# philres/ngmlr

Measured on AMD Instinct MI355X. Metric: aligned Gbp/hour (PacBio 10kb synthetic, convex-gap SW hot path, host buffers in -> results out, CIGAR bit-exact), higher is better.
Workload: dtype f32

## Files before the change

### include/cvx_align.h

```cpp
#ifndef CVX_ALIGN_H
#define CVX_ALIGN_H

#include <stdint.h>
#include <stddef.h>

#ifdef __cplusplus
extern "C" {
#endif

#define CVX_ABI_VERSION 9

enum {
	CVX_OK = 0,
	CVX_ERR_NO_DEVICE = -1,
	CVX_ERR_PARAMS = -2,
	CVX_ERR_ARG = -3,
	CVX_ERR_OOM = -4,
	CVX_ERR_HIP = -5,
	CVX_ERR_CAPACITY = -6
};

enum {
	CVX_TILE_OK = 0,
	CVX_TILE_INVALID_ROW0 = 1,
// ... 109 lines not shown

int cvx_batch_upload(cvx_handle h, int32_t n_tiles, const cvx_tile *tiles, cvx_batch *out);
int cvx_batch_run(cvx_handle h, cvx_batch b);
int cvx_batch_timing(cvx_batch b, cvx_timing *t);
int cvx_batch_ops_total(cvx_batch b, uint64_t *n_ops);
int cvx_batch_launch_info(cvx_batch b, int32_t i, cvx_launch_info *info);
int cvx_batch_download(cvx_handle h, cvx_batch b, cvx_result *results,
		uint32_t *ops_arena, uint64_t ops_capacity, uint64_t *ops_used);
void cvx_batch_free(cvx_handle h, cvx_batch b);

int cvx_submit(cvx_handle h, int32_t n_tiles, const cvx_tile *tiles, cvx_job *out);
int cvx_wait(cvx_handle h, cvx_job job, const cvx_result **results, const uint32_t **ops, uint64_t *n_ops);
int cvx_job_poll(cvx_handle h, cvx_job job, int32_t *done);
int cvx_job_timing(cvx_job job, cvx_timing *t);
int cvx_job_launch_info(cvx_job job, int32_t i, cvx_launch_info *info);
void cvx_job_release(cvx_handle h, cvx_job job);

int cvx_host_alloc(uint64_t bytes, void **out);
void cvx_host_free(void *p);

int cvx_corridor_rows(cvx_handle h, const cvx_tile *tile, int32_t *offset, int32_t *length);

int cvx_pack_probe(int32_t n_tiles, const cvx_tile *tiles, int32_t iters, int32_t assume_page_locked, double *ms_per_iter, uint64_t *bytes_touched);

typedef struct cvx_genome_s *cvx_genome;
uint64_t cvx_genome_encoded_bytes(int32_t n, const uint64_t *lengths);
int cvx_genome_encode(int32_t n, const char *const *seqs, const uint64_t *lengths, uint8_t *bin_ref,
		uint64_t *n_nibbles, uint64_t *start_table, int32_t *n_starts);
int cvx_genome_upload(cvx_handle h, const uint8_t *bin_ref, uint64_t n_nibbles, const uint64_t *start_table,
		int32_t n_starts, cvx_genome *out);
// ... 173 lines not shown
```

### ngmlr_amd/capi.py

```python
from __future__ import annotations

import ctypes as C
import os

HERE = os.path.dirname(os.path.abspath(__file__))
LIB_PATH = os.environ.get("CVX_LIB") or os.path.join(HERE, "libcvxalign.so")

CVX_OK = 0
STAGE_SCORE, STAGE_DECODE, STAGE_SEARCH = 0, 1, 2
ERR_NAMES = {0: "CVX_OK", -1: "CVX_ERR_NO_DEVICE", -2: "CVX_ERR_PARAMS", -3: "CVX_ERR_ARG",
             -4: "CVX_ERR_OOM", -5: "CVX_ERR_HIP", -6: "CVX_ERR_CAPACITY"}
TILE_STATUS = {0: "ok", 1: "invalid-row0", 2: "invalid-edge", 3: "invalid-length", 4: "too-large",
               5: "empty", -1: "unsupported"}

EXPORTS = ("cvx_last_error", "cvx_abi_version", "cvx_source_id", "cvx_device_count", "cvx_device_synchronize", "cvx_create", "cvx_destroy",
           "cvx_align_batch", "cvx_batch_upload", "cvx_batch_run", "cvx_batch_timing",
           "cvx_batch_ops_total", "cvx_batch_launch_info", "cvx_batch_download", "cvx_batch_free",
           "cvx_submit", "cvx_wait", "cvx_job_timing", "cvx_job_launch_info", "cvx_job_release",
           "cvx_format_alignment", "cvx_format_batch", "cvx_score_batch",
           "cvx_genome_encoded_bytes", "cvx_genome_encode", "cvx_genome_upload", "cvx_genome_free",
           "cvx_genome_decode", "cvx_submit_windows", "cvx_job_text",
           "cvx_host_alloc", "cvx_host_free", "cvx_corridor_rows", "cvx_pack_probe", "cvx_build_id", "cvx_job_poll", "cvx_score_kernel_ms",
           "cvx_index_upload", "cvx_index_free", "cvx_search_batch", "cvx_search_batch_ex", "cvx_job_nm_profile", "cvx_job_nm_profile_resident", "cvx_job_text_all", "cvx_job_window_refs", "cvx_job_nm_sizes", "cvx_nm_profile_ops",
           "cvx_job_nm_regions", "cvx_nm_regions_ops", "cvx_nm_regions_host",
           "cvx_sam_record_text", "cvx_sam_unmapped_text", "cvx_sam_batch", "cvx_stage_kernel_ms", "cvx_search_last_attempts", "cvx_index_build", "cvx_index_build_device",
           "cvx_corridor_fit", "cvx_corridor_fit_batch", "cvx_create_ex", "cvx_runtime_regime", "cvx_search_batch_arena",
           "cvx_score_submit", "cvx_score_poll", "cvx_score_wait")


class CvxParams(C.Structure):
    _fields_ = [("match", C.c_float), ("mismatch", C.c_float), ("gap_open", C.c_float),
                ("gap_extend", C.c_float), ("gap_extend_min", C.c_float), ("gap_decay", C.c_float)]

# ... 114 lines not shown
    lib.cvx_batch_upload.argtypes = [C.c_void_p, C.c_int32, C.POINTER(CvxTile), C.POINTER(C.c_void_p)]
    lib.cvx_batch_run.argtypes = [C.c_void_p, C.c_void_p]
    lib.cvx_batch_timing.argtypes = [C.c_void_p, C.POINTER(CvxTiming)]
    lib.cvx_batch_launch_info.argtypes = [C.c_void_p, C.c_int32, C.POINTER(CvxLaunchInfo)]
    lib.cvx_batch_ops_total.argtypes = [C.c_void_p, C.POINTER(C.c_uint64)]
    lib.cvx_batch_download.argtypes = [C.c_void_p, C.c_void_p, C.POINTER(CvxResult), C.c_void_p,
                                       C.c_uint64, C.POINTER(C.c_uint64)]
    lib.cvx_batch_free.argtypes = [C.c_void_p, C.c_void_p]
    lib.cvx_batch_free.restype = None
    lib.cvx_submit.argtypes = [C.c_void_p, C.c_int32, C.POINTER(CvxTile), C.POINTER(C.c_void_p)]
    lib.cvx_wait.argtypes = [C.c_void_p, C.c_void_p, C.POINTER(C.POINTER(CvxResult)), C.POINTER(C.POINTER(C.c_uint32)),
                             C.POINTER(C.c_uint64)]
    lib.cvx_job_poll.argtypes = [C.c_void_p, C.c_void_p, C.POINTER(C.c_int32)]
    lib.cvx_job_timing.argtypes = [C.c_void_p, C.POINTER(CvxTiming)]
    lib.cvx_job_launch_info.argtypes = [C.c_void_p, C.c_int32, C.POINTER(CvxLaunchInfo)]
    lib.cvx_job_release.argtypes = [C.c_void_p, C.c_void_p]
    lib.cvx_job_release.restype = None
    lib.cvx_format_batch.argtypes = [C.c_int32, C.POINTER(CvxResult), C.c_void_p, C.POINTER(CvxTile),
                                     C.POINTER(CvxTextBuffers), C.POINTER(CvxAlignmentText), C.c_int32]
    lib.cvx_genome_encoded_bytes.restype = C.c_uint64
    lib.cvx_genome_encoded_bytes.argtypes = [C.c_int32, C.c_void_p]
    lib.cvx_genome_encode.argtypes = [C.c_int32, C.POINTER(C.c_char_p), C.c_void_p, C.c_void_p, C.POINTER(C.c_uint64),
                                      C.c_void_p, C.POINTER(C.c_int32)]
    lib.cvx_genome_upload.argtypes = [C.c_void_p, C.c_void_p, C.c_uint64, C.c_void_p, C.c_int32, C.POINTER(C.c_void_p)]
    lib.cvx_genome_free.argtypes = [C.c_void_p, C.c_void_p]
    lib.cvx_genome_free.restype = None
    lib.cvx_genome_decode.argtypes = [C.c_void_p, C.c_void_p, C.c_int32, C.c_void_p, C.c_void_p, C.c_void_p, C.c_void_p]
    lib.cvx_submit_windows.argtypes = [C.c_void_p, C.c_void_p, C.c_int32, C.POINTER(CvxTile), C.c_void_p, C.POINTER(C.c_void_p)]
    lib.cvx_job_text.argtypes = [C.c_void_p, C.c_void_p, C.c_void_p, C.c_void_p, C.POINTER(CvxAlignmentText), C.c_void_p,
                                 C.POINTER(C.c_char_p), C.POINTER(C.c_uint64)]
# ... 67 lines not shown
```

### ngmlr_amd/csrc/cvx_host_logic.h

```cpp
#ifndef CVX_HOST_LOGIC_H
#define CVX_HOST_LOGIC_H

#include <algorithm>
#include <cmath>
#include <condition_variable>
#include <cstdlib>
#include <cstring>
#include <deque>
#include <functional>
#include <mutex>
#include <system_error>
#include <thread>
#include <vector>

#include <pthread.h>

#include "cvx_align.h"
#include "cvx_types.h"

namespace cvx {


struct KernelClass {
	int m;
// ... 523 lines not shown
		hp.n_fast++;
		hp.cls[(size_t) k * 2 + (wrap ? 1 : 0)].push_back(i);
	}
	for (size_t slot = 0; slot < per_tile.size(); ++slot) {
		size_t deepest = 0;
		for (auto &v : per_tile[slot]) deepest = std::max(deepest, v.size());
		for (size_t g = 0; g < deepest; ++g)
			for (auto &v : per_tile[slot])
				if (g < v.size()) hp.chain_tasks[slot].push_back(v[g]);
	}
	for (auto &v : hp.cls) lpt_sort(v, plan);
}



struct ScheduleTuning {
	int exact_steps = kExactDirectSteps;
	int bt_group = 0;
	bool bt_per_class = true;
	bool overlap_post = false;
	int wide_prio = 1, gang_prio = 0, chain_prio = -1, chain_lds_kb = 48;
};

enum { kModeTwoPhase = 0, kModeExact = 1, kModeChain = 2 };

enum StreamSlot { kOnSide0 = 0, kOnPost = 1, kOnMain = 2, kOnSide1 = 3, kStreamSlots = 4 };

struct WalkPlan { int n_long = 0, long_lanes = 32, bulk_lanes = 64; };

inline WalkPlan walk_plan(int count, int n_walk, int bt_group, uint64_t mean_h, const int32_t *list, const TileIn *tin) {
	const int auto_group = count <= 6144 ? 64 : count <= 12288 ? 32 : count <= 49152 ? 16 : 8;
	WalkPlan w;
	w.bulk_lanes = bt_group > 0 ? bt_group : bt_group < 0 ? (n_walk < 4096 ? 64 : 8) : auto_group;
	if (bt_group <= 0 && w.bulk_lanes <= 16)
		while (w.n_long < count && (uint64_t) tin[(size_t) list[w.n_long]].H > 3 * mean_h) w.n_long++;
	return w;
}

inline size_t chain_pad_lds(uint64_t live, int num_cus, int chain_lds_kb, bool rings_beside) {
	const uint64_t resident = std::min<uint64_t>(8192, std::max<uint64_t>(768, live + live / 2 + 256));
	const size_t per_cu = (size_t) ((resident + (uint64_t) num_cus - 1) / (uint64_t) num_cus);
	size_t pad_lds = per_cu >= 32 ? 0 : (size_t) (160 * 1024) / per_cu - 4096;
	pad_lds = std::min<size_t>(pad_lds, 60 * 1024) / 256 * 256;
	if (rings_beside && chain_lds_kb > 0 && per_cu > 0 && per_cu < 32) {
		const size_t budget = (size_t) chain_lds_kb * 1024 / per_cu;
		const size_t capped = budget > 4096 ? (budget - 4096) / 256 * 256 : 0;
		pad_lds = std::min(pad_lds, capped);
	}
	return pad_lds;
}

// ... 7 lines not shown
	size_t pad_lds = 0;
	int prio = 0;
	int stream = kOnMain;
	size_t bt_off = 0;
	int bt_count = 0;
	WalkPlan walk;
	cvx_launch_info info;
};

struct ComputeSchedule {
	std::vector<FillLaunch> launches;
	size_t n_listed = 0;
	size_t bt_begin = 0;
	int n_walk = 0;
	bool per_class = false;
	WalkPlan walk;
	size_t chain_task_off[kNumChainClasses * 2] = {0}, chain_tile_off[kNumChainClasses * 2] = {0};
	size_t chain_blk_off = 0, chain_bytes = 0;
};

inline void build_schedule(HostPlan &hp, const TilePlan *plan, const TileIn *tin, int n, uint64_t n_rows, int num_cus,
		const ScheduleTuning &t, int32_t *lists, ComputeSchedule &s) {
	size_t n_listed = 0;
	size_t cls_off[kNumClasses * 2];
	int n_direct[kNumClasses * 2];
	int ring_classes = 0;
	for (size_t c = 0; c < hp.cls.size(); ++c) {
		std::vector<int32_t> &v = hp.cls[c];
		cls_off[c] = n_listed;
		n_direct[c] = 0;
// ... 69 lines not shown
			const TileIn &in = tin[(size_t) ti];
			L.info.cells += p.cells; L.info.active_cells += p.active;
			L.info.alg_bytes += p.cells + 6ull * (uint64_t) in.H + 2ull * (uint64_t) in.W;
			L.info.read_bases += (uint64_t) in.H;
			if (!hp.trun[(size_t) ti].skip) count[(size_t) bucket(ti) + 1]++;
		}
		for (int k = 0; k < kBuckets; ++k) count[(size_t) k + 1] += count[(size_t) k];
		L.bt_off = n_listed;
		L.bt_count = count[(size_t) kBuckets];
		for (int32_t ti : *L.tiles) if (!hp.trun[(size_t) ti].skip) lists[n_listed + (size_t) count[(size_t) bucket(ti)]++] = ti;
		n_listed += (size_t) L.bt_count;
	}
	s.n_listed = n_listed;
	s.n_walk = (int) (n_listed - s.bt_begin);

	s.per_class = t.bt_per_class && s.launches.size() > 1 && !t.overlap_post && s.n_walk >= 4096;
	const uint64_t mean_h = n_rows / (uint64_t) std::max(n, 1);
	if (s.per_class) for (FillLaunch &L : s.launches) L.walk = walk_plan(L.bt_count, s.n_walk, t.bt_group, mean_h, lists + L.bt_off, tin);
	else s.walk = walk_plan(s.n_walk, s.n_walk, t.bt_group, mean_h, lists + s.bt_begin, tin);

	s.chain_blk_off = s.chain_bytes = 0;
	if (hp.n_chained) {
		for (size_t c = 0; c < hp.chain_tasks.size(); ++c) { s.chain_task_off[c] = s.chain_bytes; s.chain_bytes += hp.chain_tasks[c].size() * sizeof(ChainTask); }
		s.chain_blk_off = s.chain_bytes; s.chain_bytes += hp.chain_blk.size() * sizeof(ChainBlk);
		for (size_t c = 0; c < hp.chain_tiles.size(); ++c) { s.chain_tile_off[c] = s.chain_bytes; s.chain_bytes += (hp.chain_tiles[c].size() * sizeof(int32_t) + 7) / 8 * 8; }
	}
}

}

#endif
```

### ngmlr_amd/csrc/cvx_rt.h

```cpp
#ifndef CVX_RT_H
#define CVX_RT_H

#include <hip/hip_runtime_api.h>

#include <atomic>
#include <cstdint>
#include <mutex>
#include <string>
#include <vector>

#include "cvx_align.h"
#include "cvx_host_logic.h"
#include "cvx_launch.h"
#include "cvx_nm_regions.h"
#include "cvx_rt_err.h"
#include "cvx_types.h"

using namespace cvx;

#define HIP_TRY(expr)                                                              \
	do {                                                                           \
		hipError_t e_ = (expr);                                                    \
		if (e_ != hipSuccess) {                                                    \
			set_err("%s failed: %s (%s:%d)", #expr, hipGetErrorString(e_), __FILE__, __LINE__); \
			return (e_ == hipErrorOutOfMemory) ? CVX_ERR_OOM : CVX_ERR_HIP;        \
		}                                                                          \
	} while (0)

// ... 178 lines not shown
	bool have_refs = false;
	DevBuf<WindowDesc> d_win;
	PinBuf h_chain;
	DevBuf<uint8_t> d_chain;
	DevBuf<BoundaryRec> d_bnd;
	uint32_t bnd_epoch = 0;
	DevBuf<ChainOut> d_chain_out;

	hipEvent_t ev_bt0 = nullptr, ev_bt1 = nullptr;
	hipEvent_t ev_in = nullptr;
	hipEvent_t ev_res = nullptr;
	hipEvent_t ev[5] = {nullptr, nullptr, nullptr, nullptr, nullptr};
	std::vector<hipEvent_t> lev;
	std::vector<cvx_launch_info> launches;
	cvx_timing timing;

	const TileIn *tin() const { return h_tin.as<TileIn>(); }
	const TilePlan *plan() const { return h_plan.as<TilePlan>(); }
	const ResultRec *res() const { return h_res.as<ResultRec>(); }
	const BatchSummary *summary() const { return reinterpret_cast<const BatchSummary *>(h_res.as<uint8_t>() + (size_t) n * sizeof(ResultRec)); }

	static const int kSharedMarks = 32;
	void bind(size_t *marks) {
		int k = 0;
		PinBuf *pins[] = { &h_seq, &h_delta, &h_rsrc, &h_tin, &h_plan, &h_trun, &h_tout, &h_lists, &h_res, &h_ops, &h_chain };
		for (PinBuf *b_ : pins) b_->hwm = &marks[k++];
		d_seq.hwm = &marks[k++]; d_rows.hwm = &marks[k++]; d_delta.hwm = &marks[k++]; d_rsrc.hwm = &marks[k++]; d_tin.hwm = &marks[k++];
		d_plan.hwm = &marks[k++]; d_trun.hwm = &marks[k++]; d_tout.hwm = &marks[k++]; d_dirs.hwm = &marks[k++]; d_regions.hwm = &marks[k++];
		d_lists.hwm = &marks[k++]; d_dstoff.hwm = &marks[k++]; d_dense.hwm = &marks[k++]; d_res.hwm = &marks[k++];
		d_chain.hwm = &marks[k++]; d_bnd.hwm = &marks[k++]; d_chain_out.hwm = &marks[k++];
// ... 29 lines not shown
		if (ev_res) { (void) hipEventDestroy(ev_res); ev_res = nullptr; }
		if (ev_bt0) { (void) hipEventDestroy(ev_bt0); ev_bt0 = nullptr; }
		if (ev_bt1) { (void) hipEventDestroy(ev_bt1); ev_bt1 = nullptr; }
		for (auto &e : ev) if (e) { (void) hipEventDestroy(e); e = nullptr; }
		for (auto &e : lev) if (e) (void) hipEventDestroy(e);
		lev.clear();
	}
};

struct cvx_context {
	int device = 0;
	hipStream_t s_io = nullptr;
	hipStream_t s_main = nullptr;
	hipStream_t s_text = nullptr;
	hipStream_t s_post = nullptr;
	hipStream_t aux[kAuxStreams] = {nullptr};
	bool service = false;
	bool owns_main = true;
	std::mutex streams_mtx;
	std::atomic<bool> streams_ready{false};
	hipStream_t s_main2 = nullptr, s_post2 = nullptr, aux2[kAuxStreams] = {nullptr};
	unsigned small_jobs = 0;
	ScoreParams sp;
	uint64_t max_matrix_mb = 10000;
	int num_cus = 256;
	int pack_threads = 16;
	int tune_min_slots = 0;
	int tune_late_min = kLateMinGroups;
	int tune_late_shift = kLateShift;
	int tune_max_slots = 0;
// ... 1 lines not shown
	int tune_gang_prio = 0;
	int tune_gangs = 0;
	int tune_long_steps = 0, tune_small_batch = 0;
	bool single_lane = true;
	int tune_exact_steps = kExactDirectSteps;
	int tune_wide_prio = 1;
	int tune_chain_prio = -1;
	int tune_chain_lds_kb = 48;
	int tune_chain_m = 0;
	int tune_force_wrap = 0;
	int tune_pen_table = 1;
	int test_fail_compute = 0;
	int bt_group = 0;
	bool bt_per_class = true;
	bool overlap_post = false;
	bool sse_variant = false;
	size_t marks[cvx_batch_s::kSharedMarks] = {0};
	std::vector<cvx_batch_s *> pool;
	std::vector<cvx_batch_s *> pending;
	std::vector<cvx_batch_s *> live;
	float decode_kernel_ms = 0.0f;
	bool score_no_diag = false;
	struct cvx_score_state *score = nullptr;
	struct cvx_search_state *search = nullptr;
};

struct cvx_genome_s {
	int device = 0;
	uint64_t n_nibbles = 0;
	int32_t n_starts = 0;
// ... 6 lines not shown
```

### ngmlr_amd/csrc/cvx_rt_align.cpp

```cpp
#include <algorithm>
#include <atomic>
#include <chrono>
#include <cstdio>
#include <cstdlib>
#include <cstring>
#include <new>
#include <string>
#include <vector>

#include "cvx_rt.h"

namespace {

static const size_t kPoolBatches = 8;

cvx_batch_s *acquire_batch(cvx_context *h) {
	if (!h->pool.empty()) {
		cvx_batch_s *b = h->pool.back();
		h->pool.pop_back();
		return b;
	}
	return new (std::nothrow) cvx_batch_s();
}

// ... 244 lines not shown
	a.sp = h->sp;
	ba.chain_blk = chain_blk;
	ba.n_tiles = b->n;
}

int issue_walk(cvx_batch_s *b, const BacktrackArgs &ba, const WalkPlan &w, size_t at, int count, hipStream_t ws, hipStream_t side) {
	if (count <= 0) return CVX_OK;
	const int32_t *list = b->d_lists.p + at;
	const bool fork = w.n_long > 0 && side != nullptr;
	if (fork) {
		HIP_TRY(hipEventRecord(b->ev_bt0, ws));
		HIP_TRY(hipStreamWaitEvent(side, b->ev_bt0, 0));
	}
	if (w.n_long > 0) HIP_TRY(launch_backtrack(ba, list, w.n_long, w.long_lanes, fork ? side : ws));
	if (fork) HIP_TRY(hipEventRecord(b->ev_bt1, side));
	HIP_TRY(launch_backtrack(ba, list + w.n_long, count - w.n_long, w.bulk_lanes, ws));
	if (fork) HIP_TRY(hipStreamWaitEvent(ws, b->ev_bt1, 0));
	return CVX_OK;
}

int upload_chain(cvx_batch_s *b, const HostPlan &hp, const ComputeSchedule &sch, hipStream_t st) {
	RC_TRY(b->h_chain.ensure(sch.chain_bytes));
	uint8_t *hc = b->h_chain.as<uint8_t>();
	for (size_t c = 0; c < hp.chain_tasks.size(); ++c)
		if (!hp.chain_tasks[c].empty()) memcpy(hc + sch.chain_task_off[c], hp.chain_tasks[c].data(), hp.chain_tasks[c].size() * sizeof(ChainTask));
	memcpy(hc + sch.chain_blk_off, hp.chain_blk.data(), hp.chain_blk.size() * sizeof(ChainBlk));
	for (size_t c = 0; c < hp.chain_tiles.size(); ++c)
		if (!hp.chain_tiles[c].empty()) memcpy(hc + sch.chain_tile_off[c], hp.chain_tiles[c].data(), hp.chain_tiles[c].size() * sizeof(int32_t));
	RC_TRY(b->d_chain.ensure(sch.chain_bytes));
	RC_TRY(b->d_chain_out.ensure(hp.chain_blk.size()));
	{
		const size_t had = b->d_bnd.cap;
		RC_TRY(b->d_bnd.ensure((size_t) hp.bnd_recs + 64));
		if (b->d_bnd.cap != had || b->bnd_epoch >= kBndEpochMax) {
			HIP_TRY(hipMemsetAsync(b->d_bnd.p, 0, b->d_bnd.cap * sizeof(BoundaryRec), st));
			b->bnd_epoch = 0;
		}
		b->bnd_epoch += 1;
	}
	HIP_TRY(hipMemcpyAsync(b->d_chain.p, hc, sch.chain_bytes, hipMemcpyHostToDevice, st));
	return CVX_OK;
}

int stage_compute(cvx_context *h, cvx_batch_s *b, bool streaming = false) {
	const int n = b->n;
	if (h->test_fail_compute > 0 && --h->test_fail_compute == 0) {
		set_err("stage_compute: failure injected by CVX_TUNE_FAIL_COMPUTE");
		return CVX_ERR_OOM;
	}
	const bool second = streaming && n > 0 && n < kSmallJobTiles && !h->single_lane && ((h->small_jobs++ & 1u) != 0u);
	hipStream_t const S_main = second ? h->s_main2 : h->s_main;
	hipStream_t const S_post = second ? h->s_post2 : h->s_post;
	hipStream_t const *S_aux = second ? h->aux2 : h->aux;
	b->s_run = S_main;
	hipStream_t st = S_main;
	HIP_TRY(hipEventSynchronize(b->ev_in));
	b->launches.clear();
	b->ops_total = 0;
	b->have_ops = false;
	if (n == 0) {
		HIP_TRY(hipEventRecord(b->ev[4], st));
		hipStream_t ps = h->overlap_post ? S_post : S_main;
		HIP_TRY(hipStreamWaitEvent(ps, b->ev[4], 0));
		HIP_TRY(hipEventRecord(b->ev[2], ps));
		HIP_TRY(hipEventRecord(b->ev[3], ps));
		HIP_TRY(hipEventRecord(b->ev_res, ps));
		b->state = kComputed;
		return CVX_OK;
	}

	HostPlan hp;
	PlanTuning tune;
	tune.min_slots = h->tune_min_slots; tune.max_slots = h->tune_max_slots; tune.force_wrap = h->tune_force_wrap; tune.chain_m = h->tune_chain_m;
	tune.force_generic = h->sse_variant ? 1 : 0;
// ... 5 lines not shown
		expand_rows_host(rsrc[(size_t) i], b->tin()[(size_t) i].H, b->h_delta.as<uint8_t>(), b->h_rowsx.as<RowDesc>(), tmp.data());
		return tmp.data();
	}, true, tune, hp);
	const std::vector<int32_t> &generic = hp.generic;
	RC_TRY(b->d_dirs.ensure((size_t) hp.dir_dwords + 64));
	RC_TRY(b->d_regions.ensure((size_t) hp.ops_ints + 64));
	b->dense_cap = std::min<uint64_t>(hp.ops_ints, hp.ops_ints / 3 + 64ull * (uint64_t) n);
	RC_TRY(b->d_dense.ensure((size_t) b->dense_cap + 64));
	b->dense_cap = std::max<uint64_t>(b->dense_cap, b->d_dense.cap - 64);

	RC_TRY(b->h_trun.ensure((size_t) n * sizeof(TileRun)));
	RC_TRY(b->h_tout.ensure((size_t) n * sizeof(TileOut)));
	RC_TRY(b->h_lists.ensure((size_t) 2 * n * sizeof(int32_t) + 64));
	ScheduleTuning stune;
	stune.exact_steps = h->tune_exact_steps; stune.bt_group = h->bt_group; stune.bt_per_class = h->bt_per_class; stune.overlap_post = h->overlap_post;
	stune.wide_prio = h->tune_wide_prio; stune.gang_prio = h->tune_gang_prio; stune.chain_prio = h->tune_chain_prio; stune.chain_lds_kb = h->tune_chain_lds_kb;
	ComputeSchedule sch;
	build_schedule(hp, b->plan(), b->tin(), n, b->n_rows, h->num_cus, stune, b->h_lists.as<int32_t>(), sch);
	memcpy(b->h_trun.p, hp.trun.data(), (size_t) n * sizeof(TileRun));
	memcpy(b->h_tout.p, hp.tout.data(), (size_t) n * sizeof(TileOut));
	if (!generic.empty()) {
		RC_TRY(b->h_goff.ensure((generic.size() + 1) * sizeof(uint64_t)));
		uint64_t *goff = b->h_goff.as<uint64_t>();
		goff[0] = 0;
		for (size_t g = 0; g < generic.size(); ++g)
			goff[g + 1] = goff[g] + (uint64_t) generic_scratch_bytes(hp.trun[(size_t) generic[g]].ring);
		RC_TRY(b->d_gscratch.ensure((size_t) goff[generic.size()] + 256));
		RC_TRY(b->d_gscratch_off.ensure(generic.size() + 1));
		HIP_TRY(hipMemcpyAsync(b->d_gscratch_off.p, goff, (generic.size() + 1) * sizeof(uint64_t), hipMemcpyHostToDevice, st));
	}
// ... 43 lines not shown
			HIP_TRY(hipEventRecord(le[kLevTwoPhase], ls));
		} else {
			a.list = b->d_lists.p + L.list_off;
			a.list_n = L.n_direct;
			if (a.list_n > 0) HIP_TRY(launch_fill(L.m, L.gang, wrap, kModeExact, a, 0, ls));
			a.list += L.n_direct;
			a.list_n = L.count - L.n_direct;
			if (a.list_n > 0) HIP_TRY(launch_fill(L.m, L.gang, wrap, kModeTwoPhase, a, 0, ls));
			HIP_TRY(hipEventRecord(le[kLevTwoPhase], ls));
			if (a.list_n > 0) HIP_TRY(launch_fill(L.m, L.gang, wrap, kModeExact, a, 0, ls));
		}
		HIP_TRY(hipEventRecord(le[kLevExact], ls));
		if (sch.per_class) RC_TRY(issue_walk(b, ba, L.walk, L.bt_off, L.bt_count, ls, nullptr));
		HIP_TRY(hipEventRecord(le[kLevWalked], ls));
	}
	st = h->overlap_post ? S_post : S_main;
	HIP_TRY(hipStreamWaitEvent(st, b->ev[4], 0));
	for (int i = 0; i < launches; ++i) HIP_TRY(hipStreamWaitEvent(st, b->lev[(size_t) i * kLevPerLaunch + kLevWalked], 0));
	HIP_TRY(hipEventRecord(b->ev[2], st));

	if (!sch.per_class) RC_TRY(issue_walk(b, ba, sch.walk, sch.bt_begin, sch.n_walk, st, S_aux[0]));
	ResultRec *d_rec = reinterpret_cast<ResultRec *>(b->d_res.p);
	BatchSummary *d_sum = reinterpret_cast<BatchSummary *>(b->d_res.p + (size_t) n * sizeof(ResultRec));
	HIP_TRY(launch_finalize(b->d_tout.p, b->d_plan.p, b->d_dstoff.p, d_rec, d_sum, b->d_counters.p, n, b->dense_cap, st));
	HIP_TRY(launch_compact(b->d_regions.p, b->d_trun.p, b->d_tout.p, b->d_dstoff.p, b->d_dense.p, n, b->dense_cap, st));
	HIP_TRY(hipEventRecord(b->ev[3], st));
	HIP_TRY(hipMemcpyAsync(b->h_res.p, b->d_res.p, (size_t) n * sizeof(ResultRec) + sizeof(BatchSummary), hipMemcpyDeviceToHost, st));
	HIP_TRY(hipEventRecord(b->ev_res, st));

	b->timing.cells = hp.cells;
	b->timing.active_cells = hp.active;
	b->timing.dir_bytes = hp.dir_dwords * 4;
	b->timing.n_fill_launches = launches;
	b->timing.n_tiles_fast = hp.n_fast;
	b->timing.n_tiles_chained = hp.n_chained;
	b->state = kComputed;
	return CVX_OK;
}

int stage_results(cvx_context *h, cvx_batch_s *b) {
// ... 13 lines not shown
	b->timing.backtrack_ms = std::max(0.0f, ev_ms(b->ev[4], b->ev[3]) - fill_end);
	b->timing.total_ms = b->timing.plan_ms + ev_ms(b->ev[4], b->ev[3]);
	b->timing.n_tiles_redone = s->n_redone;
	b->timing.chain_task_ticks = s->chain_task_ticks;
	b->timing.chain_poll_ticks = s->chain_poll_ticks;
	b->state = kFinished;
	return CVX_OK;
}

int stage_ops(cvx_context *h, cvx_batch_s *b) {
	if (b->have_ops) return CVX_OK;
	if (b->ops_total > b->dense_cap) {
		const uint64_t cap = b->ops_total;
		RC_TRY(b->d_dense.ensure((size_t) cap + 64));
		b->dense_cap = b->d_dense.cap - 64;
		hipStream_t ps = b->s_run ? b->s_run : h->s_main;
		HIP_TRY(launch_compact(b->d_regions.p, b->d_trun.p, b->d_tout.p, b->d_dstoff.p, b->d_dense.p, b->n, b->dense_cap, ps));
		HIP_TRY(hipStreamSynchronize(ps));
	}
	if (b->ops_total) {
		RC_TRY(b->h_ops.ensure((size_t) b->ops_total * sizeof(uint32_t)));
		HIP_TRY(hipMemcpyAsync(b->h_ops.p, b->d_dense.p, (size_t) b->ops_total * sizeof(uint32_t), hipMemcpyDeviceToHost, h->s_io));
		HIP_TRY(hipStreamSynchronize(h->s_io));
	}
	b->have_ops = true;
	return CVX_OK;
}

int pump(cvx_context *h, bool block, const cvx_batch_s *upto) {
	while (!h->pending.empty()) {
		cvx_batch_s *b = h->pending.front();
		if (!block) {
			hipError_t q = hipEventQuery(b->ev_in);
			if (q == hipErrorNotReady) { (void) hipGetLastError(); break; }
			if (q != hipSuccess) { set_err("hipEventQuery: %s", hipGetErrorString(q)); h->pending.erase(h->pending.begin()); (void) fail_job(b, CVX_ERR_HIP); continue; }
		}
		h->pending.erase(h->pending.begin());
		const int rc = stage_compute(h, b, true);
		if (rc != CVX_OK) (void) fail_job(b, rc);
		if (upto && b == upto) break;
	}
	return CVX_OK;
}

}

extern "C" {


int cvx_batch_upload(cvx_handle h, int32_t n, const cvx_tile *tiles, cvx_batch *out) {
	ABI_GUARD_BEGIN
	if (!h || !out || n < 0 || (n > 0 && !tiles)) { set_err("cvx_batch_upload: bad argument"); return CVX_ERR_ARG; }
	*out = nullptr;
// ... 8 lines not shown
	if (rc != CVX_OK) { discard_batch(h, b); return rc; }
	*out = b;
	return CVX_OK;
	ABI_GUARD_END
}

int cvx_batch_run(cvx_handle h, cvx_batch b) {
	ABI_GUARD_BEGIN
	if (!h || !b || b->state < kUploaded) { set_err("cvx_batch_run: NULL argument / batch not uploaded"); return CVX_ERR_ARG; }
	HIP_TRY(hipSetDevice(h->device));
	RC_TRY(stage_plan(h, b, h->s_main));
	RC_TRY(stage_compute(h, b));
	RC_TRY(stage_results(h, b));
	HIP_TRY(hipStreamSynchronize(h->s_main));
	HIP_TRY(hipStreamSynchronize(h->s_post));
	return CVX_OK;
	ABI_GUARD_END
}

int cvx_batch_timing(cvx_batch b, cvx_timing *t) {
	ABI_GUARD_BEGIN
	if (!b || !t) { set_err("cvx_batch_timing: NULL argument"); return CVX_ERR_ARG; }
	*t = b->timing;
	return CVX_OK;
	ABI_GUARD_END
}

int cvx_batch_launch_info(cvx_batch b, int32_t i, cvx_launch_info *info) {
	ABI_GUARD_BEGIN
	if (!b || !info || b->state < kFinished || i < 0 || (size_t) i >= b->launches.size()) { set_err("cvx_batch_launch_info: bad index"); return CVX_ERR_ARG; }
// ... 147 lines not shown
	*done = 0;
	if (j->state == kFailed || j->state >= kFinished) { *done = 1; return CVX_OK; }
	if (j->state >= kComputed) {
		hipError_t q = hipEventQuery(j->ev_res);
		if (q == hipSuccess) *done = 1;
		else if (q == hipErrorNotReady) (void) hipGetLastError();
		else { set_err("hipEventQuery: %s", hipGetErrorString(q)); return CVX_ERR_HIP; }
	}
	return CVX_OK;
	ABI_GUARD_END
}

int cvx_job_timing(cvx_job j, cvx_timing *t) { ABI_GUARD_BEGIN return cvx_batch_timing(j, t); ABI_GUARD_END }
int cvx_job_launch_info(cvx_job j, int32_t i, cvx_launch_info *info) { ABI_GUARD_BEGIN return cvx_batch_launch_info(j, i, info); ABI_GUARD_END }

void cvx_job_release(cvx_handle h, cvx_job j) {
	ABI_GUARD_BEGIN
	if (!j) return;
	if (h) {
		(void) hipSetDevice(h->device);
		auto it = std::find(h->pending.begin(), h->pending.end(), j);
		if (it != h->pending.end()) h->pending.erase(it);
		if ((j->state >= kPlanned && j->state < kFinished) || j->state == kFailed) (void) hipDeviceSynchronize();
	}
	recycle_batch(h, j);
	ABI_GUARD_END_VOID
}


int cvx_corridor_rows(cvx_handle h, const cvx_tile *tile, int32_t *offset, int32_t *length) {
// ... 86 lines not shown
```

### ngmlr_amd/csrc/cvx_runtime.cpp

```cpp
#include <hip/hip_runtime_api.h>
#include <dirent.h>
#include <unistd.h>

#include <algorithm>
#include <atomic>
#include <cmath>
#include <cstdarg>
#include <cstdio>
#include <cstdlib>
#include <cstring>
#include <functional>
#include <mutex>
#include <new>
#include <string>
#include <vector>

#include "cvx_rt.h"

namespace {

static const int kServiceStreamsMax = 16, kMaxServiceDevices = 64;
struct ServiceStreams { hipStream_t st[kServiceStreamsMax] = {nullptr}; unsigned next = 0; };
ServiceStreams g_service_streams[kMaxServiceDevices];
std::mutex g_service_mtx;
// ... 34 lines not shown

int ensure_streams(cvx_context *c) {
	if (c->streams_ready.load(std::memory_order_acquire)) return CVX_OK;
	std::lock_guard<std::mutex> lk(c->streams_mtx);
	if (c->streams_ready.load(std::memory_order_relaxed)) return CVX_OK;
	int prio_lo = 0, prio_hi = 0;
	(void) hipDeviceGetStreamPriorityRange(&prio_lo, &prio_hi);
	hipError_t e = hipSuccess;
	auto make = [&](hipStream_t *st) { if (e == hipSuccess && *st == nullptr) e = hipStreamCreateWithFlags(st, hipStreamNonBlocking); };
	make(&c->s_post);
	{
		const char *tp = getenv("CVX_TEXT_STREAM_PRIO");
		if (e == hipSuccess && c->s_text == nullptr && !(tp && atoi(tp) == 0)) e = hipStreamCreateWithPriority(&c->s_text, hipStreamNonBlocking, prio_hi);
	}
	make(&c->s_text);
	for (int i = 0; i < kAuxStreams; ++i) make(&c->aux[i]);
	make(&c->s_main2);
	make(&c->s_post2);
	for (int i = 0; i < kAuxStreams; ++i) make(&c->aux2[i]);
	if (e == hipSuccess) e = hipStreamCreateWithPriority(&c->s_io, hipStreamNonBlocking, prio_hi);
	if (e != hipSuccess) { set_err("hipStreamCreate failed: %s", hipGetErrorString(e)); return CVX_ERR_HIP; }
	c->streams_ready.store(true, std::memory_order_release);
	return CVX_OK;
}

}

namespace cvx {
void pack_pool_run(int n_tasks, const std::function<void(int)> &fn) { PackPool::get().run(n_tasks, fn); }
}
// ... 121 lines not shown
	if (strncmp(prop.gcnArchName, "gfx950", 6) != 0) {
		set_err("cvx_create: device %d is %s; this library carries gfx950 code only", device_id, prop.gcnArchName);
		return CVX_ERR_NO_DEVICE;
	}
	cvx_context *c = new (std::nothrow) cvx_context();
	if (!c) return CVX_ERR_OOM;
	c->device = device_id;
	c->num_cus = prop.multiProcessorCount > 0 ? prop.multiProcessorCount : 256;
	c->sp.mat = p->match; c->sp.mis = p->mismatch; c->sp.go = p->gap_open;
	c->sp.ge = p->gap_extend; c->sp.gem = p->gap_extend_min; c->sp.decay = p->gap_decay;
	c->max_matrix_mb = max_matrix_mb ? max_matrix_mb : 10000;
	c->sse_variant = !fast_regime;
	if (const char *e = getenv("CVX_TUNE_BT_GROUP")) c->bt_group = atoi(e);
	if (const char *e = getenv("CVX_TUNE_BT_PER_CLASS")) c->bt_per_class = atoi(e) != 0;
	if (const char *e = getenv("CVX_TUNE_OVERLAP_POST")) c->overlap_post = atoi(e) != 0;
	if (const char *e = getenv("CVX_TUNE_SSE_VARIANT")) c->sse_variant = c->sse_variant || atoi(e) != 0;
	c->pack_threads = PackPool::get().size();
	if (const char *e = getenv("CVX_TUNE_MIN_M")) c->tune_min_slots = atoi(e);
	if (const char *e = getenv("CVX_TUNE_FORCE_WRAP16")) c->tune_force_wrap = atoi(e);
	if (const char *e = getenv("CVX_TUNE_PEN_TABLE")) c->tune_pen_table = atoi(e) != 0;
	{
		volatile float prod = (float) kPenClamp * p->gap_decay;
		volatile float at_clamp = p->gap_extend + prod;
		const bool reached = !(at_clamp < p->gap_extend_min);
		if (!(p->gap_decay >= 0.0f) || !(reached || p->gap_decay == 0.0f)) c->tune_pen_table = 0;
	}
	if (const char *e = getenv("CVX_TUNE_FAIL_COMPUTE")) c->test_fail_compute = atoi(e);
	if (const char *e = getenv("CVX_TUNE_SCORE_NO_DIAG")) c->score_no_diag = atoi(e) != 0;
	if (const char *e = getenv("CVX_TUNE_MAX_M")) c->tune_max_slots = atoi(e);
	if (const char *e = getenv("CVX_TUNE_CHAIN_M")) c->tune_chain_m = atoi(e);
// ... 34 lines not shown
		return CVX_ERR_HIP;
	}
	*out = c;
	return CVX_OK;
	ABI_GUARD_END
}

void cvx_destroy(cvx_handle h) {
	ABI_GUARD_BEGIN
	if (!h) return;
	(void) hipSetDevice(h->device);
	(void) hipDeviceSynchronize();
	g_deferred.drain();
	if (h->s_main && h->owns_main) (void) hipStreamDestroy(h->s_main);
	if (h->s_post) (void) hipStreamDestroy(h->s_post);
	if (h->s_text) (void) hipStreamDestroy(h->s_text);
	if (h->s_io) (void) hipStreamDestroy(h->s_io);
	for (auto &a : h->aux) if (a) (void) hipStreamDestroy(a);
	if (h->s_main2) (void) hipStreamDestroy(h->s_main2);
	if (h->s_post2) (void) hipStreamDestroy(h->s_post2);
	for (auto &a : h->aux2) if (a) (void) hipStreamDestroy(a);
	for (cvx_batch_s *b : h->pool) { b->release(); delete b; }
	h->pool.clear();
	for (cvx_batch_s *b : h->live) { b->release(); delete b; }
	h->live.clear();
	h->pending.clear();
	score_state_free(h->score);
	search_state_free(h->search);
	delete h;
	ABI_GUARD_END_VOID
// ... 36 lines not shown
```

Before: 15940.

## Add one-tile-per-lane backtrack walk on a dedicated stream for streamed follower batches

Adds a new backtrack kernel in which each lane of a 64-wide wavefront walks one tile's traceback on its own. It is used for large streaming follower batches and runs on a new high-priority walk stream, with a grid-bounded strided compaction kernel after it. The pump can now hold a leader batch back while the previous batch's fills are still in flight, so the lane walk and compaction can overlap the next batch's fill work. The cost is heavy lane divergence and per-lane scattered memory reads in the walk. The extra stream and scheduling conditions also add complexity and new ordering paths.

```diff
diff --git a/include/cvx_align.h b/include/cvx_align.h
--- a/include/cvx_align.h
+++ b/include/cvx_align.h
@@ -147,6 +147,7 @@
 int cvx_job_poll(cvx_handle h, cvx_job job, int32_t *done);
 int cvx_job_timing(cvx_job job, cvx_timing *t);
 int cvx_job_launch_info(cvx_job job, int32_t i, cvx_launch_info *info);
+int cvx_job_walk_lanes(cvx_job job, int32_t *lanes);
 void cvx_job_release(cvx_handle h, cvx_job job);
 
 int cvx_host_alloc(uint64_t bytes, void **out);
diff --git a/ngmlr_amd/capi.py b/ngmlr_amd/capi.py
--- a/ngmlr_amd/capi.py
+++ b/ngmlr_amd/capi.py
@@ -16,7 +16,7 @@
 EXPORTS = ("cvx_last_error", "cvx_abi_version", "cvx_source_id", "cvx_device_count", "cvx_device_synchronize", "cvx_create", "cvx_destroy",
            "cvx_align_batch", "cvx_batch_upload", "cvx_batch_run", "cvx_batch_timing",
            "cvx_batch_ops_total", "cvx_batch_launch_info", "cvx_batch_download", "cvx_batch_free",
-           "cvx_submit", "cvx_wait", "cvx_job_timing", "cvx_job_launch_info", "cvx_job_release",
+           "cvx_submit", "cvx_wait", "cvx_job_timing", "cvx_job_launch_info", "cvx_job_walk_lanes", "cvx_job_release",
            "cvx_format_alignment", "cvx_format_batch", "cvx_score_batch",
            "cvx_genome_encoded_bytes", "cvx_genome_encode", "cvx_genome_upload", "cvx_genome_free",
            "cvx_genome_decode", "cvx_submit_windows", "cvx_job_text",
@@ -161,6 +161,8 @@
     lib.cvx_job_poll.argtypes = [C.c_void_p, C.c_void_p, C.POINTER(C.c_int32)]
     lib.cvx_job_timing.argtypes = [C.c_void_p, C.POINTER(CvxTiming)]
     lib.cvx_job_launch_info.argtypes = [C.c_void_p, C.c_int32, C.POINTER(CvxLaunchInfo)]
+    if hasattr(lib, "cvx_job_walk_lanes"):
+        lib.cvx_job_walk_lanes.argtypes = [C.c_void_p, C.POINTER(C.c_int32)]
     lib.cvx_job_release.argtypes = [C.c_void_p, C.c_void_p]
     lib.cvx_job_release.restype = None
     lib.cvx_format_batch.argtypes = [C.c_int32, C.POINTER(CvxResult), C.c_void_p, C.POINTER(CvxTile),
diff --git a/ngmlr_amd/csrc/cvx_host_logic.h b/ngmlr_amd/csrc/cvx_host_logic.h
--- a/ngmlr_amd/csrc/cvx_host_logic.h
+++ b/ngmlr_amd/csrc/cvx_host_logic.h
@@ -561,12 +561,18 @@
 
 
 
+static const int kLaneWalkMinTiles = 16384;
+static const int kLaneWalkMaxSteps = 32768;
+
 struct ScheduleTuning {
 	int exact_steps = kExactDirectSteps;
 	int bt_group = 0;
 	bool bt_per_class = true;
 	bool overlap_post = false;
 	int wide_prio = 1, gang_prio = 0, chain_prio = -1, chain_lds_kb = 48;
+	bool streaming = false, follower = false;
+	bool lane_walk = true;
+	int lane_min = kLaneWalkMinTiles;
 };
 
 enum { kModeTwoPhase = 0, kModeExact = 1, kModeChain = 2 };
@@ -582,6 +588,12 @@
 	if (bt_group <= 0 && w.bulk_lanes <= 16)
 		while (w.n_long < count && (uint64_t) tin[(size_t) list[w.n_long]].H > 3 * mean_h) w.n_long++;
 	return w;
+}
+
+inline bool lane_walk_chosen(const ScheduleTuning &t, int n_walk, int max_steps) {
+	if (t.bt_group == 1) return true;
+	if (!t.lane_walk || t.bt_group != 0) return false;
+	return t.streaming && t.follower && n_walk >= t.lane_min && n_walk > 0 && max_steps <= kLaneWalkMaxSteps;
 }
 
 inline size_t chain_pad_lds(uint64_t live, int num_cus, int chain_lds_kb, bool rings_beside) {
@@ -619,6 +631,8 @@
 	size_t bt_begin = 0;
 	int n_walk = 0;
 	bool per_class = false;
+	bool lane_walk = false;
+	int max_steps = 0;
 	WalkPlan walk;
 	size_t chain_task_off[kNumChainClasses * 2] = {0}, chain_tile_off[kNumChainClasses * 2] = {0};
 	size_t chain_blk_off = 0, chain_bytes = 0;
@@ -718,10 +732,14 @@
 	s.n_listed = n_listed;
 	s.n_walk = (int) (n_listed - s.bt_begin);
 
-	s.per_class = t.bt_per_class && s.launches.size() > 1 && !t.overlap_post && s.n_walk >= 4096;
+	s.max_steps = 0;
+	for (size_t i = s.bt_begin; i < n_listed; ++i) s.max_steps = std::max(s.max_steps, (int) hp.trun[(size_t) lists[i]].nsteps);
+	s.lane_walk = lane_walk_chosen(t, s.n_walk, s.max_steps);
+	s.per_class = t.bt_per_class && s.launches.size() > 1 && !t.overlap_post && s.n_walk >= 4096 && !s.lane_walk;
 	const uint64_t mean_h = n_rows / (uint64_t) std::max(n, 1);
 	if (s.per_class) for (FillLaunch &L : s.launches) L.walk = walk_plan(L.bt_count, s.n_walk, t.bt_group, mean_h, lists + L.bt_off, tin);
 	else s.walk = walk_plan(s.n_walk, s.n_walk, t.bt_group, mean_h, lists + s.bt_begin, tin);
+	if (s.lane_walk) { s.walk.bulk_lanes = 1; s.walk.n_long = 0; }
 
 	s.chain_blk_off = s.chain_bytes = 0;
 	if (hp.n_chained) {
diff --git a/ngmlr_amd/csrc/cvx_launch_walk.h b/ngmlr_amd/csrc/cvx_launch_walk.h
--- /dev/null
+++ b/ngmlr_amd/csrc/cvx_launch_walk.h
@@ -0,0 +1,16 @@
+#ifndef CVX_LAUNCH_WALK_H
+#define CVX_LAUNCH_WALK_H
+
+#include <hip/hip_runtime_api.h>
+#include <stdint.h>
+
+#include "cvx_types.h"
+
+namespace cvx {
+
+hipError_t launch_backtrack_lanes(const BacktrackArgs &a, const int32_t *order, int n_order, hipStream_t st);
+hipError_t launch_compact_bounded(const int32_t *regions, const TileRun *trun, const TileOut *tout,
+		const uint64_t *dst_off, uint32_t *dense, int n_tiles, uint64_t dense_cap, int max_groups, hipStream_t st);
+
+}
+#endif
diff --git a/ngmlr_amd/csrc/cvx_rt.h b/ngmlr_amd/csrc/cvx_rt.h
--- a/ngmlr_amd/csrc/cvx_rt.h
+++ b/ngmlr_amd/csrc/cvx_rt.h
@@ -12,6 +12,7 @@
 #include "cvx_align.h"
 #include "cvx_host_logic.h"
 #include "cvx_launch.h"
+#include "cvx_launch_walk.h"
 #include "cvx_nm_regions.h"
 #include "cvx_rt_err.h"
 #include "cvx_types.h"
@@ -220,6 +221,9 @@
 	std::vector<hipEvent_t> lev;
 	std::vector<cvx_launch_info> launches;
 	cvx_timing timing;
+	int compact_groups = 0;
+	hipStream_t s_post_run = nullptr;
+	int walk_lanes = 0;
 
 	const TileIn *tin() const { return h_tin.as<TileIn>(); }
 	const TilePlan *plan() const { return h_plan.as<TilePlan>(); }
@@ -279,6 +283,7 @@
 	hipStream_t s_main = nullptr;
 	hipStream_t s_text = nullptr;
 	hipStream_t s_post = nullptr;
+	hipStream_t s_walk = nullptr;
 	hipStream_t aux[kAuxStreams] = {nullptr};
 	bool service = false;
 	bool owns_main = true;
@@ -310,6 +315,9 @@
 	int bt_group = 0;
 	bool bt_per_class = true;
 	bool overlap_post = false;
+	bool lane_walk = true;
+	int lane_min = kLaneWalkMinTiles;
+	bool lane_hold = false;
 	bool sse_variant = false;
 	size_t marks[cvx_batch_s::kSharedMarks] = {0};
 	std::vector<cvx_batch_s *> pool;
diff --git a/ngmlr_amd/csrc/cvx_rt_align.cpp b/ngmlr_amd/csrc/cvx_rt_align.cpp
--- a/ngmlr_amd/csrc/cvx_rt_align.cpp
+++ b/ngmlr_amd/csrc/cvx_rt_align.cpp
@@ -282,8 +282,17 @@
 	}
 	if (w.n_long > 0) HIP_TRY(launch_backtrack(ba, list, w.n_long, w.long_lanes, fork ? side : ws));
 	if (fork) HIP_TRY(hipEventRecord(b->ev_bt1, side));
-	HIP_TRY(launch_backtrack(ba, list + w.n_long, count - w.n_long, w.bulk_lanes, ws));
+	if (w.bulk_lanes == 1) HIP_TRY(launch_backtrack_lanes(ba, list + w.n_long, count - w.n_long, ws));
+	else HIP_TRY(launch_backtrack(ba, list + w.n_long, count - w.n_long, w.bulk_lanes, ws));
 	if (fork) HIP_TRY(hipStreamWaitEvent(ws, b->ev_bt1, 0));
+	return CVX_OK;
+}
+
+int issue_compact(cvx_batch_s *b, hipStream_t st) {
+	if (b->compact_groups > 0)
+		HIP_TRY(launch_compact_bounded(b->d_regions.p, b->d_trun.p, b->d_tout.p, b->d_dstoff.p, b->d_dense.p, b->n, b->dense_cap, b->compact_groups, st));
+	else
+		HIP_TRY(launch_compact(b->d_regions.p, b->d_trun.p, b->d_tout.p, b->d_dstoff.p, b->d_dense.p, b->n, b->dense_cap, st));
 	return CVX_OK;
 }
 
@@ -310,7 +319,7 @@
 	return CVX_OK;
 }
 
-int stage_compute(cvx_context *h, cvx_batch_s *b, bool streaming = false) {
+int stage_compute(cvx_context *h, cvx_batch_s *b, bool streaming = false, bool follower = false) {
 	const int n = b->n;
 	if (h->test_fail_compute > 0 && --h->test_fail_compute == 0) {
 		set_err("stage_compute: failure injected by CVX_TUNE_FAIL_COMPUTE");
@@ -321,11 +330,13 @@
 	hipStream_t const S_post = second ? h->s_post2 : h->s_post;
 	hipStream_t const *S_aux = second ? h->aux2 : h->aux;
 	b->s_run = S_main;
+	b->s_post_run = nullptr;
 	hipStream_t st = S_main;
 	HIP_TRY(hipEventSynchronize(b->ev_in));
 	b->launches.clear();
 	b->ops_total = 0;
 	b->have_ops = false;
+	b->walk_lanes = 0;
 	if (n == 0) {
 		HIP_TRY(hipEventRecord(b->ev[4], st));
 		hipStream_t ps = h->overlap_post ? S_post : S_main;
@@ -361,6 +372,7 @@
 	RC_TRY(b->h_lists.ensure((size_t) 2 * n * sizeof(int32_t) + 64));
 	ScheduleTuning stune;
 	stune.exact_steps = h->tune_exact_steps; stune.bt_group = h->bt_group; stune.bt_per_class = h->bt_per_class; stune.overlap_post = h->overlap_post;
+	stune.streaming = streaming; stune.follower = follower; stune.lane_walk = h->lane_walk; stune.lane_min = h->lane_min;
 	stune.wide_prio = h->tune_wide_prio; stune.gang_prio = h->tune_gang_prio; stune.chain_prio = h->tune_chain_prio; stune.chain_lds_kb = h->tune_chain_lds_kb;
 	ComputeSchedule sch;
 	build_schedule(hp, b->plan(), b->tin(), n, b->n_rows, h->num_cus, stune, b->h_lists.as<int32_t>(), sch);
@@ -434,7 +446,11 @@
 		if (sch.per_class) RC_TRY(issue_walk(b, ba, L.walk, L.bt_off, L.bt_count, ls, nullptr));
 		HIP_TRY(hipEventRecord(le[kLevWalked], ls));
 	}
-	st = h->overlap_post ? S_post : S_main;
+	const bool on_post = h->overlap_post || sch.lane_walk;
+	b->walk_lanes = sch.per_class ? (launches ? sch.launches[0].walk.bulk_lanes : 0) : sch.walk.bulk_lanes;
+	b->compact_groups = sch.lane_walk ? 4 * h->num_cus : 0;
+	st = sch.lane_walk ? h->s_walk : on_post ? S_post : S_main;
+	b->s_post_run = st;
 	HIP_TRY(hipStreamWaitEvent(st, b->ev[4], 0));
 	for (int i = 0; i < launches; ++i) HIP_TRY(hipStreamWaitEvent(st, b->lev[(size_t) i * kLevPerLaunch + kLevWalked], 0));
 	HIP_TRY(hipEventRecord(b->ev[2], st));
@@ -443,7 +459,7 @@
 	ResultRec *d_rec = reinterpret_cast<ResultRec *>(b->d_res.p);
 	BatchSummary *d_sum = reinterpret_cast<BatchSummary *>(b->d_res.p + (size_t) n * sizeof(ResultRec));
 	HIP_TRY(launch_finalize(b->d_tout.p, b->d_plan.p, b->d_dstoff.p, d_rec, d_sum, b->d_counters.p, n, b->dense_cap, st));
-	HIP_TRY(launch_compact(b->d_regions.p, b->d_trun.p, b->d_tout.p, b->d_dstoff.p, b->d_dense.p, n, b->dense_cap, st));
+	RC_TRY(issue_compact(b, st));
 	HIP_TRY(hipEventRecord(b->ev[3], st));
 	HIP_TRY(hipMemcpyAsync(b->h_res.p, b->d_res.p, (size_t) n * sizeof(ResultRec) + sizeof(BatchSummary), hipMemcpyDeviceToHost, st));
 	HIP_TRY(hipEventRecord(b->ev_res, st));
@@ -487,8 +503,8 @@
 		const uint64_t cap = b->ops_total;
 		RC_TRY(b->d_dense.ensure((size_t) cap + 64));
 		b->dense_cap = b->d_dense.cap - 64;
-		hipStream_t ps = b->s_run ? b->s_run : h->s_main;
-		HIP_TRY(launch_compact(b->d_regions.p, b->d_trun.p, b->d_tout.p, b->d_dstoff.p, b->d_dense.p, b->n, b->dense_cap, ps));
+		hipStream_t ps = b->s_post_run ? b->s_post_run : b->s_run ? b->s_run : h->s_main;
+		RC_TRY(issue_compact(b, ps));
 		HIP_TRY(hipStreamSynchronize(ps));
 	}
 	if (b->ops_total) {
@@ -498,6 +514,18 @@
 	}
 	b->have_ops = true;
 	return CVX_OK;
+}
+
+bool fills_in_flight(const cvx_context *h, const cvx_batch_s *b) {
+	const cvx_batch_s *prev = nullptr;
+	for (const cvx_batch_s *j : h->live) {
+		if (j == b) break;
+		if (j->state == kComputed && j->n > 0) prev = j;
+	}
+	if (!prev) return false;
+	const hipError_t q = hipEventQuery(prev->ev[2]);
+	if (q == hipErrorNotReady) { (void) hipGetLastError(); return true; }
+	return false;
 }
 
 int pump(cvx_context *h, bool block, const cvx_batch_s *upto) {
@@ -508,8 +536,10 @@
 			if (q == hipErrorNotReady) { (void) hipGetLastError(); break; }
 			if (q != hipSuccess) { set_err("hipEventQuery: %s", hipGetErrorString(q)); h->pending.erase(h->pending.begin()); (void) fail_job(b, CVX_ERR_HIP); continue; }
 		}
+		const bool follower = h->pending.size() > 1;
+		if (!block && !follower && h->lane_walk && h->bt_group == 0 && b->n >= h->lane_min && (h->lane_hold || fills_in_flight(h, b))) break;
 		h->pending.erase(h->pending.begin());
-		const int rc = stage_compute(h, b, true);
+		const int rc = stage_compute(h, b, true, follower);
 		if (rc != CVX_OK) (void) fail_job(b, rc);
 		if (upto && b == upto) break;
 	}
@@ -548,6 +578,7 @@
 	RC_TRY(stage_results(h, b));
 	HIP_TRY(hipStreamSynchronize(h->s_main));
 	HIP_TRY(hipStreamSynchronize(h->s_post));
+	if (h->s_walk) HIP_TRY(hipStreamSynchronize(h->s_walk));
 	return CVX_OK;
 	ABI_GUARD_END
 }
@@ -725,6 +756,14 @@
 int cvx_job_timing(cvx_job j, cvx_timing *t) { ABI_GUARD_BEGIN return cvx_batch_timing(j, t); ABI_GUARD_END }
 int cvx_job_launch_info(cvx_job j, int32_t i, cvx_launch_info *info) { ABI_GUARD_BEGIN return cvx_batch_launch_info(j, i, info); ABI_GUARD_END }
 
+int cvx_job_walk_lanes(cvx_job j, int32_t *lanes) {
+	ABI_GUARD_BEGIN
+	if (!j || !lanes || j->state < kFinished) { set_err("cvx_job_walk_lanes: job not finished (call cvx_wait first)"); return CVX_ERR_ARG; }
+	*lanes = j->walk_lanes;
+	return CVX_OK;
+	ABI_GUARD_END
+}
+
 void cvx_job_release(cvx_handle h, cvx_job j) {
 	ABI_GUARD_BEGIN
 	if (!j) return;
diff --git a/ngmlr_amd/csrc/cvx_runtime.cpp b/ngmlr_amd/csrc/cvx_runtime.cpp
--- a/ngmlr_amd/csrc/cvx_runtime.cpp
+++ b/ngmlr_amd/csrc/cvx_runtime.cpp
@@ -72,6 +72,7 @@
 		if (e == hipSuccess && c->s_text == nullptr && !(tp && atoi(tp) == 0)) e = hipStreamCreateWithPriority(&c->s_text, hipStreamNonBlocking, prio_hi);
 	}
 	make(&c->s_text);
+	if (e == hipSuccess && c->s_walk == nullptr) e = hipStreamCreateWithPriority(&c->s_walk, hipStreamNonBlocking, prio_hi);
 	for (int i = 0; i < kAuxStreams; ++i) make(&c->aux[i]);
 	make(&c->s_main2);
 	make(&c->s_post2);
@@ -223,6 +224,9 @@
 	if (const char *e = getenv("CVX_TUNE_BT_GROUP")) c->bt_group = atoi(e);
 	if (const char *e = getenv("CVX_TUNE_BT_PER_CLASS")) c->bt_per_class = atoi(e) != 0;
 	if (const char *e = getenv("CVX_TUNE_OVERLAP_POST")) c->overlap_post = atoi(e) != 0;
+	if (const char *e = getenv("CVX_TUNE_LANE_WALK")) c->lane_walk = atoi(e) != 0;
+	if (const char *e = getenv("CVX_TUNE_LANE_HOLD")) c->lane_hold = atoi(e) != 0;
+	if (const char *e = getenv("CVX_TUNE_LANE_MIN")) c->lane_min = std::max(1, atoi(e));
 	if (const char *e = getenv("CVX_TUNE_SSE_VARIANT")) c->sse_variant = c->sse_variant || atoi(e) != 0;
 	c->pack_threads = PackPool::get().size();
 	if (const char *e = getenv("CVX_TUNE_MIN_M")) c->tune_min_slots = atoi(e);
@@ -287,6 +291,7 @@
 	g_deferred.drain();
 	if (h->s_main && h->owns_main) (void) hipStreamDestroy(h->s_main);
 	if (h->s_post) (void) hipStreamDestroy(h->s_post);
+	if (h->s_walk) (void) hipStreamDestroy(h->s_walk);
 	if (h->s_text) (void) hipStreamDestroy(h->s_text);
 	if (h->s_io) (void) hipStreamDestroy(h->s_io);
 	for (auto &a : h->aux) if (a) (void) hipStreamDestroy(a);
diff --git a/ngmlr_amd/csrc/cvx_walk_lane.hip b/ngmlr_amd/csrc/cvx_walk_lane.hip
--- /dev/null
+++ b/ngmlr_amd/csrc/cvx_walk_lane.hip
@@ -0,0 +1,175 @@
+#include <hip/hip_runtime.h>
+#include <stdint.h>
+
+#include "cvx_types.h"
+#include "cvx_launch_walk.h"
+
+namespace cvx {
+
+#define CVX_DEV __device__ __forceinline__
+
+CVX_DEV void valid_bounds(const int off, const int width, int &minC, int &maxC) {
+	minC = (int) ((float) off + 0.1f * (float) width);
+	maxC = (int) ((float) (minC + width) - 0.1f * (float) width);
+}
+
+CVX_DEV unsigned plane_code(const unsigned wx, const unsigned wy, const int bit) {
+	const unsigned px = (wx >> bit) & 1u, py = (wy >> bit) & 1u;
+	return px ? (py ? 1u : 2u) : (py ? 3u : 0u);
+}
+
+__global__ void __launch_bounds__(64)
+backtrack_lane_kernel(const BacktrackArgs a, const int32_t *order, const int n_order) {
+	__builtin_amdgcn_s_setprio(3);
+	const int q = blockIdx.x * 64 + threadIdx.x;
+	bool has = q < n_order;
+	const int t = has ? (order ? order[q] : q) : 0;
+	TileOut o;
+	o.score = -1.0f; o.status = 0; o.best_x = 0; o.best_y = 0;
+	o.ref_position = 0; o.qstart = 0; o.qend = 0; o.n_ops = 0; o.ops_first = 0; o.pad = 0;
+	TileRun tr;
+	TileIn ti;
+	tr.skip = 1; tr.ring = 64; tr.r0 = 0; tr.ops_cap = 8; tr.dir_off = 0; tr.ops_off = 0; tr.chain_blk0 = -1;
+	ti.H = 0; ti.W = 0; ti.row_off = 0; ti.ref_off = 0; ti.qry_off = 0;
+	if (has) {
+		tr = a.trun[t];
+		o = a.tout[t];
+		ti = a.tin[t];
+		if (tr.skip != 0 || o.status != 0 || o.pad != 0) has = false;
+	}
+	const int H = ti.H, W = ti.W;
+	const RowView rows = row_view(a.rsrc[t], a.rows, ti.row_off);
+	bool dead = false;
+	if (has && !(o.score > 0.0f)) {
+		int fy = -1, fx = 0;
+		for (int yy = 0; yy < H && fy < 0; ++yy) {
+			const RowDesc2 ol = row_at(rows, yy);
+			long long lo = ol.x > 0 ? ol.x : 0;
+			long long hi = (long long) ol.x + (long long) ol.y;
+			if (hi > W) hi = W;
+			if (hi > lo) { fy = yy; fx = (int) lo; }
+		}
+		if (fy < 0) { dead = true; has = false; }
+		else { o.score = 0.0f; o.best_x = fx; o.best_y = fy; }
+	}
+	const bool chained = tr.chain_blk0 >= 0;
+	const int N = tr.ring, r0 = tr.r0, ops_cap = tr.ops_cap;
+	const ChainBlk *blk = a.chain_blk + (chained ? tr.chain_blk0 : 0);
+	const uint2 *dirs = reinterpret_cast<const uint2 *>(a.dirs);
+	const size_t dbase = chained ? (size_t) 0 : (size_t) (tr.dir_off >> 1);
+	const uint32_t *seq32 = reinterpret_cast<const uint32_t *>(a.seq);
+	int *ops = a.ops + tr.ops_off;
+
+	const int best_x = o.best_x, best_y = o.best_y;
+	bool act = has;
+	if (has && best_y <= 0) { o.status = 1; act = false; }
+	const bool walked = act;
+	const int qend = (H - best_y) - 1;
+	int idx = ops_cap - 1;
+	int elem = 4;
+	int elem_len = qend;
+	int consumed = qend;
+	int x = best_x, y = best_y;
+	int s = act ? y % N : 0;
+	int status = 0;
+	int budget = 2 * (best_x + best_y) + 8;
+
+	size_t c_widx = ~(size_t) 0;
+	uint2 w = make_uint2(0u, 0u);
+	int c_y = -1, minC = 0, maxC = 0;
+	RowDesc2 ol; ol.x = 0; ol.y = 0;
+	int c_lo = 0, c_hi = 0;
+	ChainBlk c_cb;
+	c_cb.dir_off = 0; c_cb.tblk0 = 0; c_cb.nblk32 = 1;
+	uint32_t c_rw = 0xffffffffu, c_qw = 0xffffffffu, rword = 0u, qword = 0u;
+
+	while (__builtin_amdgcn_ballot_w64(act) != 0ull) {
+		if (act) {
+			if (--budget < 0) { status = 3; act = false; }
+			else {
+				const bool inside = (x >= 0 && y >= 0);
+				const int lx = x > 0 ? x : 0, ly = y > 0 ? y : 0;
+				const int tt = x + y - r0;
+				const int ttc = tt > 0 ? tt : 0;
+				size_t widx;
+				if (chained) {
+					if (ly < c_lo || ly >= c_hi) { const int gb = ly / N; c_lo = gb * N; c_hi = c_lo + N; c_cb = blk[gb]; }
+					int wr = (ttc >> 5) - c_cb.tblk0;
+					wr = wr < 0 ? 0 : (wr >= c_cb.nblk32 ? c_cb.nblk32 - 1 : wr);
+					widx = c_cb.dir_off + (size_t) wr * N + (size_t) (ly - c_lo);
+				} else {
+					widx = dbase + (size_t) (ttc >> 5) * N + s;
+				}
+				if (widx != c_widx) { w = dirs[widx]; c_widx = widx; }
+				if (ly != c_y) { ol = row_at(rows, ly); c_y = ly; valid_bounds(ol.x, ol.y, minC, maxC); }
+				const uint32_t ra = ti.ref_off + (uint32_t) lx, qa = ti.qry_off + (uint32_t) ly;
+				if ((ra >> 2) != c_rw) { c_rw = ra >> 2; rword = seq32[c_rw]; }
+				if ((qa >> 2) != c_qw) { c_qw = qa >> 2; qword = seq32[c_qw]; }
+				const bool in_row = inside && tt >= 0 && x >= ol.x && x < ol.x + ol.y;
+				unsigned code = plane_code(w.x, w.y, 31 - (ttc & 31));
+				if (!in_row) code = 0u;
+				if (code == 0u) act = false;
+				else if (!(x > minC && x < maxC)) { status = 2; act = false; }
+				else {
+					const unsigned rc = (rword >> ((ra & 3u) * 8u)) & 0xffu, qc = (qword >> ((qa & 3u) * 8u)) & 0xffu;
+					const int cur = code == 3u ? (rc == qc ? 7 : 8) : (int) code;
+					if (cur == elem) elem_len += 1;
+					else {
+						if (elem != 4) { if (idx >= 0) ops[idx] = (elem_len << 4) | elem; idx -= 1; }
+						elem = cur;
+						elem_len = 1;
+					}
+					if (code != 1u) x -= 1;
+					if (code != 2u) { y -= 1; consumed += 1; s -= 1; if (s < 0) s += N; }
+				}
+			}
+		}
+	}
+	if (walked) {
+		if (status == 0) {
+			if (elem != 4) { if (idx >= 0) ops[idx] = (elem_len << 4) | elem; idx -= 1; }
+			consumed += (y + 1);
+			o.ref_position = x + 1;
+			o.qstart = y + 1;
+			o.qend = qend;
+			o.ops_first = idx + 1;
+			o.n_ops = ops_cap - 1 - idx;
+			if (H != consumed || idx < -1) status = 3;
+		}
+		o.status = status;
+	}
+	if (dead) { o.score = -1.0f; o.status = 5; }
+	if (has || dead) { o.pad = 1; a.tout[t] = o; }
+}
+
+__global__ void __launch_bounds__(256)
+compact_ops_strided_kernel(const int32_t *regions, const TileRun *trun, const TileOut *tout,
+		const uint64_t *dst_off, uint32_t *dense, int n_tiles, unsigned long long dense_cap) {
+	for (int t = blockIdx.x; t < n_tiles; t += gridDim.x) {
+		const TileOut o = tout[t];
+		if (o.status != 0 || o.n_ops <= 0) continue;
+		const unsigned long long d0 = dst_off[t];
+		if (d0 + (unsigned long long) o.n_ops > dense_cap) continue;
+		const int32_t *src = regions + trun[t].ops_off + o.ops_first;
+		uint32_t *dst = dense + d0;
+		for (int i = threadIdx.x; i < o.n_ops; i += blockDim.x) dst[i] = (uint32_t) src[i];
+	}
+}
+
+hipError_t launch_backtrack_lanes(const BacktrackArgs &a, const int32_t *order, int n_order, hipStream_t st) {
+	if (a.n_tiles <= 0) return hipSuccess;
+	const int nb = order != nullptr ? n_order : a.n_tiles;
+	if (nb <= 0) return hipSuccess;
+	hipLaunchKernelGGL(backtrack_lane_kernel, dim3((nb + 63) / 64), dim3(64), 0, st, a, order, nb);
+	return hipGetLastError();
+}
+
+hipError_t launch_compact_bounded(const int32_t *regions, const TileRun *trun, const TileOut *tout,
+		const uint64_t *dst_off, uint32_t *dense, int n_tiles, uint64_t dense_cap, int max_groups, hipStream_t st) {
+	if (n_tiles <= 0) return hipSuccess;
+	hipLaunchKernelGGL(compact_ops_strided_kernel, dim3(n_tiles < max_groups ? n_tiles : (max_groups > 0 ? max_groups : 1)), dim3(256), 0, st,
+			regions, trun, tout, dst_off, dense, n_tiles, (unsigned long long) dense_cap);
+	return hipGetLastError();
+}
+
+}
```

Measured after the change: 15620. 2.0% lower.
